# bdaiinstitute/vlfm

Measured on NVIDIA H100. Metric: value-map steps/sec (ITM+cone-fuse), higher is better.
Workload: dtype f16

## Files before the change

### include/vlfm_b200.h

```cpp
#ifndef VLFM_B200_H_
#define VLFM_B200_H_

#include <stddef.h>
#include <stdint.h>

#ifdef __cplusplus
extern "C" {
#endif

#define VLFM_OK 0
#define VLFM_E_INVALID 1
#define VLFM_E_CUDA 2
#define VLFM_E_UNSUPPORTED 3
#define VLFM_E_DRIVER 4

#define VLFM_ST_CAMERA_OFF_GRID 1
#define VLFM_ST_SCATTER_OOB 2
#define VLFM_ST_FRONTIER_OVERFLOW 4

#define VLFM_FUSE_WEIGHTED 0
#define VLFM_FUSE_MAX_CONFIDENCE 1
#define VLFM_FUSE_REPLACE 2
#define VLFM_FUSE_EQUAL 4

// ... 70 lines not shown

int vlfm_preprocess_im2col(const uint8_t* d_img, uint8_t* d_mid, void* d_out, int B, int H, int W, int OH,
                           int OW, int patch, int ldk, const int32_t* d_hbounds, const int32_t* d_hkk,
                           int hksize, const int32_t* d_vbounds, const int32_t* d_vkk, int vksize,
                           const float* h_mean3, const float* h_std3, void* stream);
int vlfm_assemble_tokens(const float* d_patch, const float* d_cls, const float* d_pos, float* d_x, int B,
                         int T, int D, void* stream);
int vlfm_layernorm(const float* d_x, const float* d_gamma, const float* d_beta, void* d_out16, float* d_out32,
                   int rows, int D, int ldx, int ldo16, int ldo32, float eps, void* stream);
int vlfm_attention_f16(const void* d_q, const void* d_k, const void* d_v, void* d_o, int B, int heads, int Nq,
                       int Nk, int hd, int ldq, int ldk, int ldv, int ldo, float scale, void* stream);
#define VLFM_EPI_BIAS_GELU_F16X2 6
#define VLFM_EPI_BIAS_SILU_F16 7
int vlfm_gemm_f16x2(const void* d_A_hi, const void* d_A_lo, const void* d_W_hi, const void* d_W_lo, const float* d_bias, void* d_out,
                    void* d_out_lo, int M, int N, int K, int lda, int ldw, int ldo, int epilogue, void* stream);
int vlfm_gemm_f16x2_resid_ln(const void* d_A_hi, const void* d_A_lo, const void* d_W_hi, const void* d_W_lo, const float* d_bias,
                             float* d_x, int M, int N, int K, int lda, int ldw, int ldx, const float* d_gamma, const float* d_beta,
                             void* d_out_hi, void* d_out_lo, int ld16, float* d_out32, int ld32, float eps, float* d_partials,
                             size_t partial_bytes, void* stream);
int vlfm_layernorm_x2(const float* d_x, const float* d_gamma, const float* d_beta, void* d_out_hi, void* d_out_lo, float* d_out32,
                      int rows, int D, int ldx, int ldo16, int ldo32, float eps, void* stream);
int vlfm_layernorm_reduce_x2(float* d_x, const float* d_partials, int splits, long long split_stride, const float* d_gamma,
                             const float* d_beta, void* d_out_hi, void* d_out_lo, float* d_out32, int rows, int D, int ldx, int ldo16,
                             int ldo32, float eps, void* stream);
int vlfm_split_x2(const float* d_src, void* d_hi, void* d_lo, long long n, void* stream);
int vlfm_attention_f32(const float* d_q, const float* d_k, const float* d_v, void* d_o_hi, void* d_o_lo, int B, int heads, int Nq,
                       int Nk, int hd, int ldq, int ldk, int ldv, int ldo, float scale, void* stream);
int vlfm_itc_head(const float* d_proj, const float* d_text, float* d_out, int B, int Q, int D, void* stream);
int vlfm_itc_head_multi(const float* d_proj, const float* d_text, float* d_out, int B, int P, int Q, int D, int ldo, void* stream);
int vlfm_im2col_f16(const void* d_x16, int ldx, void* d_col16, int B, int H, int W, int C, int k, int stride, int ldk, void* stream);
// ... 137 lines not shown
```

### vlfm_b200/_lib.py

```python
from __future__ import annotations

import ctypes as C
import os

_HERE = os.path.dirname(os.path.abspath(__file__))
LIB_PATH = os.path.join(_HERE, "libvlfm_b200.so")

VLFM_OK = 0
ST_CAMERA_OFF_GRID = 1
ST_SCATTER_OOB = 2
ST_FRONTIER_OVERFLOW = 4
FUSE_WEIGHTED, FUSE_MAX_CONFIDENCE, FUSE_REPLACE, FUSE_EQUAL = 0, 1, 2, 4
EPI_BIAS_F16, EPI_BIAS_GELU_F16, EPI_BIAS_RESID_F32, EPI_BIAS_F32, EPI_BIAS_RELU_F16 = 0, 1, 2, 3, 4
EPI_BIAS_GELU_F16X2 = 6
EPI_BIAS_SILU_F16 = 7
EPI_CLUSTER_SPLIT = 256
DRAW_LINE, DRAW_CIRCLE, DRAW_RECORD_INTS = 0, 1, 8


class ValueParams(C.Structure):
    _fields_ = [
        ("H", C.c_int32), ("W", C.c_int32), ("G", C.c_int32), ("C", C.c_int32), ("R", C.c_int32),
        ("ppm", C.c_int32), ("depth_scale", C.c_float), ("depth_offset", C.c_float),
        ("decision_threshold", C.c_float), ("fusion", C.c_int32), ("rows_per_tile", C.c_int32),
# ... 37 lines not shown
    "vlfm_cast_f32_f16": (C.c_int, [_P, _P, C.c_long, _P]),
    "vlfm_cast_addpos_f16": (C.c_int, [_P, _P, _P, _P, C.c_long, _P]),
    "vlfm_msda_fused": (C.c_int, [_P, _P, C.c_int, C.c_int, _P, C.c_int, _P, C.c_int, C.c_int, C.c_int, C.c_int, C.c_int, C.c_int, _P, _P]),
    "vlfm_holes_workspace_bytes": (C.c_int, [C.c_int, C.c_int, C.POINTER(C.c_size_t)]),
    "vlfm_fill_small_holes": (C.c_int, [_P, C.c_int, C.c_int, C.c_double, _P, _P, _P, _P]),
    "vlfm_gemm_f16": (C.c_int, [_P, _P, _P, _P, C.c_int, C.c_int, C.c_int, C.c_int, C.c_int, C.c_int, C.c_int, _P]),
    "vlfm_gemm_csplit_plan": (C.c_int, [C.c_int, C.c_int, C.c_int, _P, _P, _P]),
    "vlfm_gemm_f16_resid_ln": (C.c_int, [_P, _P, _P, _P] + [C.c_int] * 6 + [_P, _P, _P, C.c_int, _P, C.c_int, C.c_float, _P, C.c_size_t, _P]),
    "vlfm_layernorm_reduce": (C.c_int, [_P, _P, C.c_int, C.c_longlong, _P, _P, _P, _P] + [C.c_int] * 5 + [C.c_float, _P]),
    "vlfm_preprocess_im2col": (C.c_int, [_P, _P, _P] + [C.c_int] * 7 + [_P, _P, C.c_int, _P, _P, C.c_int,
                                         C.POINTER(C.c_float), C.POINTER(C.c_float), _P]),
    "vlfm_assemble_tokens": (C.c_int, [_P, _P, _P, _P, C.c_int, C.c_int, C.c_int, _P]),
    "vlfm_layernorm": (C.c_int, [_P, _P, _P, _P, _P, C.c_int, C.c_int, C.c_int, C.c_int, C.c_int, C.c_float, _P]),
    "vlfm_attention_f16": (C.c_int, [_P, _P, _P, _P] + [C.c_int] * 9 + [C.c_float, _P]),
    "vlfm_gemm_f16x2": (C.c_int, [_P] * 7 + [C.c_int] * 7 + [_P]),
    "vlfm_gemm_f16x2_resid_ln": (C.c_int, [_P] * 6 + [C.c_int] * 6 + [_P, _P, _P, _P, C.c_int, _P, C.c_int, C.c_float, _P, C.c_size_t, _P]),
    "vlfm_layernorm_x2": (C.c_int, [_P] * 6 + [C.c_int] * 5 + [C.c_float, _P]),
    "vlfm_layernorm_reduce_x2": (C.c_int, [_P, _P, C.c_int, C.c_longlong, _P, _P, _P, _P, _P] + [C.c_int] * 5 + [C.c_float, _P]),
    "vlfm_split_x2": (C.c_int, [_P, _P, _P, C.c_longlong, _P]),
    "vlfm_attention_f32": (C.c_int, [_P] * 5 + [C.c_int] * 9 + [C.c_float, _P]),
    "vlfm_swin_patch_im2col": (C.c_int, [_P, _P, C.c_int, C.c_int, C.c_int, C.POINTER(C.c_float), C.POINTER(C.c_float), _P]),
    "vlfm_swin_window_attention": (C.c_int, [_P, _P, _P, _P] + [C.c_int] * 6 + [_P]),
    "vlfm_swin_patch_merge": (C.c_int, [_P, _P, C.c_int, C.c_int, C.c_int, C.c_int, _P]),
    "vlfm_explore_workspace_bytes": (C.c_int, [C.c_int, C.POINTER(C.c_size_t)]),
    "vlfm_explore_update": (C.c_int, [C.c_int, _P, _P, C.c_int, C.c_int, C.c_double, C.c_double, C.c_double, C.c_double, C.c_int, _P, _P, _P, _P, _P]),
    "vlfm_explore_env_record_bytes": (C.c_size_t, []),
    "vlfm_explore_batch_workspace_bytes": (C.c_int, [C.c_int, C.c_int, C.POINTER(C.c_size_t)]),
    "vlfm_explore_update_batch": (C.c_int, [C.c_int, C.c_int, C.POINTER(ExploreEnv), _P, _P, _P, _P, _P, _P, C.c_size_t, _P, C.c_size_t, _P]),
    "vlfm_explore_prepare_batch": (C.c_int, [C.c_int, C.c_int, C.POINTER(ExploreEnv), _P, _P, _P, _P, _P, _P, C.c_size_t, _P, C.c_size_t]),
    "vlfm_explore_launch_batch": (C.c_int, [C.c_int, C.c_int, _P, _P, _P]),
# ... 97 lines not shown
```

### vlfm_b200/csrc/gemm_wgmma.cu

```cuda
#include <cuda.h>
#include <cuda_fp16.h>
#include <math.h>
#include <stdlib.h>

#include "common.cuh"

namespace vlfm {

constexpr int BM = 128;
constexpr int BK = 64;
constexpr int GEMM_THREADS = 384;
constexpr int GEMM_CONSUMERS = 256;

__device__ __forceinline__ void mbar_expect_tx(uint32_t bar, uint32_t bytes) {
  asm volatile("mbarrier.arrive.expect_tx.shared::cta.b64 _, [%0], %1;" ::"r"(bar), "r"(bytes) : "memory");
}
__device__ __forceinline__ void mbar_arrive(uint32_t bar) {
  asm volatile("mbarrier.arrive.shared::cta.b64 _, [%0];" ::"r"(bar) : "memory");
}
__device__ __forceinline__ void tma_load_2d(uint32_t dst, const CUtensorMap* map, int x, int y, uint32_t bar) {
  asm volatile(
      "cp.async.bulk.tensor.2d.shared::cluster.global.mbarrier::complete_tx::bytes [%0], [%1, {%3, %4}], [%2];"
      ::"r"(dst), "l"(map), "r"(bar), "r"(x), "r"(y) : "memory");
}
// ... 51 lines not shown
  }
};
#undef VLFM_D16
#undef VLFM_D4

struct GemmArgs {
  const float* bias;
  void* out;
  int M, N, K, ldo, epi;
  int kb_per_split;
  long long split_stride;
  const __half* a_tail; int lda, tail_rows, tail_row0;
  void* out_lo;
  int a_box_rows;
  SplitK sk;
};
constexpr int GEMM_TAIL_MAX = 2;
static_assert(SK_SLAB_ROWS == BM + GEMM_TAIL_MAX && SK_TILE == BM, "stream-K slab = one 128 x 128 tile + its tail rows");
constexpr int GEMM_TAIL_KMAX = 6144;

__device__ __forceinline__ float gelu_erf(float x) { return 0.5f * x * (1.f + erff(x * 0.70710678118654752f)); }
__device__ __forceinline__ float silu(float x) { return x / (1.f + expf(-x)); }

__device__ __forceinline__ void epilogue_store2(const GemmArgs& g, int row, int n, float v0, float v1, bool pair, bool split) {
  const size_t idx = (size_t)row * g.ldo + n;
  if (g.epi == VLFM_EPI_BIAS_F16 || g.epi == VLFM_EPI_BIAS_GELU_F16 || g.epi == VLFM_EPI_BIAS_RELU_F16 || g.epi == VLFM_EPI_BIAS_GELU_F16X2) {
    if (g.epi == VLFM_EPI_BIAS_GELU_F16 || g.epi == VLFM_EPI_BIAS_GELU_F16X2) { v0 = gelu_erf(v0); v1 = gelu_erf(v1); }
    else if (g.epi == VLFM_EPI_BIAS_RELU_F16) { v0 = fmaxf(v0, 0.f); v1 = fmaxf(v1, 0.f); }
    __half* o = reinterpret_cast<__half*>(g.out) + idx;
    const __half2 h = __floats2half2_rn(v0, v1);
    if (pair) *reinterpret_cast<__half2*>(o) = h; else o[0] = __low2half(h);
    if (g.epi == VLFM_EPI_BIAS_GELU_F16X2) {
      const float2 f = __half22float2(h);
      const __half2 l = __floats2half2_rn((v0 - f.x) * X2_SCALE, (v1 - f.y) * X2_SCALE);
// ... 420 lines not shown
      const int rows = CS_BM + g.tail_rows, r0 = rank * rows / s_cl, r1 = (rank + 1) * rows / s_cl;
      const uint32_t base = smem_u32(part);
      for (int i = et; i < (r1 - r0) * (BN / 2); i += CS_CONSUMERS) {
        const int row = r0 + i / (BN / 2), c = (i % (BN / 2)) * 2, n = n_blk * BN + c;
        if (n >= g.N) continue;
        const uint32_t off = base + (uint32_t)(row * LDP + c) * 4;
        float2 sum = ld_peer_f2(off, 0);
        for (int p = 1; p < s_cl; ++p) { const float2 v = ld_peer_f2(off, p); sum.x += v.x; sum.y += v.y; }
        epilogue_store2(g, row, n, sum.x + sbias[c], sum.y + sbias[c + 1], n + 1 < g.N, false);
      }
    }
    cluster_sync_all();
  }
}

template <int BN, int STAGES>
__global__ void __launch_bounds__(GEMM_THREADS, 1)
gemm_f16x2_wgmma_kernel(const __grid_constant__ CUtensorMap tmA, const __grid_constant__ CUtensorMap tmAl,
                        const __grid_constant__ CUtensorMap tmB, const __grid_constant__ CUtensorMap tmBl, GemmArgs g) {
  constexpr uint32_t A_BYTES = BM * BK * 2, B_BYTES = BN * BK * 2;

  extern __shared__ uint8_t smem_raw[];
  uint8_t* sA = smem_align_1024(smem_raw);
  uint8_t* sAl = sA + STAGES * A_BYTES;
  uint8_t* sB = sAl + STAGES * A_BYTES;
  uint8_t* sBl = sB + STAGES * B_BYTES;
  uint64_t* bars = reinterpret_cast<uint64_t*>(sBl + STAGES * B_BYTES);
  const uint32_t full0 = smem_u32(bars), empty0 = smem_u32(bars + STAGES);
  float* sbias = reinterpret_cast<float*>(bars + 2 * STAGES);

  pdl_trigger();
// ... 35 lines not shown
        tma_load_2d(smem_u32(sA + s * A_BYTES), &tmA, (kb_begin + kb) * BK, m_blk * BM, full0 + 8 * s);
        tma_load_2d(smem_u32(sAl + s * A_BYTES), &tmAl, (kb_begin + kb) * BK, m_blk * BM, full0 + 8 * s);
        tma_load_2d(smem_u32(sB + s * B_BYTES), &tmB, (kb_begin + kb) * BK, n_blk * BN, full0 + 8 * s);
        tma_load_2d(smem_u32(sBl + s * B_BYTES), &tmBl, (kb_begin + kb) * BK, n_blk * BN, full0 + 8 * s);
        if (++s == STAGES) { s = 0; ph ^= 1; }
      }
    }
  } else if (warp >= 4) {
    const int wg = (warp >> 2) - 1, wq = warp & 3;
    const int et = threadIdx.x - (GEMM_THREADS - GEMM_CONSUMERS);
    const int wg_row0 = m_blk * BM + wg * 64;
    const bool active = wg_row0 < g.M;
    if (et < BN) { const int n = n_blk * BN + et; sbias[et] = (g.bias && n < g.N) ? __ldg(g.bias + n) : 0.f; }
    asm volatile("bar.sync 1, 256;" ::: "memory");
    pdl_wait();
    if (!active) {
      int s = 0; uint32_t ph = 0;
      for (int kb = 0; kb < num_k; ++kb) {
        mbar_wait(full0 + 8 * s, ph);
        __syncwarp();
        if (lane == 0) mbar_arrive(empty0 + 8 * s);
        if (++s == STAGES) { s = 0; ph ^= 1; }
      }
      return;
    }
    float acc[BN / 2], corr[BN / 2];
#pragma unroll
    for (int i = 0; i < BN / 2; ++i) { acc[i] = 0.f; corr[i] = 0.f; }
    int s = 0; uint32_t ph = 0;
    for (int kb = 0; kb < num_k; ++kb) {
      mbar_wait(full0 + 8 * s, ph);
      const uint32_t wg_off = (uint32_t)wg * (64 * BK * 2);
      const uint32_t a0 = smem_u32(sA + s * A_BYTES) + wg_off, al0 = smem_u32(sAl + s * A_BYTES) + wg_off;
      const uint32_t b0 = smem_u32(sB + s * B_BYTES), bl0 = smem_u32(sBl + s * B_BYTES);
      wg_fence();
#pragma unroll
      for (int k = 0; k < BK / 16; ++k) {
        const uint64_t da = wgmma_desc_k128(a0 + k * 32), dal = wgmma_desc_k128(al0 + k * 32);
        const uint64_t db = wgmma_desc_k128(b0 + k * 32), dbl = wgmma_desc_k128(bl0 + k * 32);
        const uint32_t first = (kb > 0 || k > 0) ? 1u : 0u;
        Wgmma<BN>::mma(acc, da, db, first);
        Wgmma<BN>::mma(corr, dal, db, first);
        Wgmma<BN>::mma(corr, da, dbl, 1u);
      }
      wg_commit();
      wg_wait<1>();
      if (kb > 0) {
        __syncwarp();
        if (lane == 0) mbar_arrive(empty0 + 8 * (s == 0 ? STAGES - 1 : s - 1));
      }
      if (++s == STAGES) { s = 0; ph ^= 1; }
    }
    wg_wait<0>();
#pragma unroll
    for (int i = 0; i < BN / 2; ++i) acc[i] = fmaf(corr[i], 1.f / X2_SCALE, acc[i]);
    epilogue_frag<BN>(acc, wg_row0 + wq * 16, n_blk, g, split, blockIdx.z == 0, sbias);
  }
}

typedef CUresult (*EncodeTiledFn)(CUtensorMap*, CUtensorMapDataType, cuuint32_t, void*, const cuuint64_t*,
                                  const cuuint64_t*, const cuuint32_t*, const cuuint32_t*, CUtensorMapInterleave,
                                  CUtensorMapSwizzle, CUtensorMapL2promotion, CUtensorMapFloatOOBfill);

static EncodeTiledFn get_encode() {
  static EncodeTiledFn fn = nullptr;
  static bool tried = false;
  if (!tried) {
    tried = true;
    void* p = nullptr;
    cudaDriverEntryPointQueryResult q;
    if (cudaGetDriverEntryPoint("cuTensorMapEncodeTiled", &p, cudaEnableDefault, &q) == cudaSuccess &&
// ... 32 lines not shown
  if (!configured) {
    rc = check_cuda(cudaFuncSetAttribute(gemm_f16_wgmma_kernel<BN, STAGES, SILU>, cudaFuncAttributeMaxDynamicSharedMemorySize, (int)smem), "cudaFuncSetAttribute(gemm)");
    if (rc) return rc;
    configured = true;
  }
  const int num_k = (g.K + BK - 1) / BK;
  dim3 grid((g.N + BN - 1) / BN, g.tail_rows > 0 ? g.M / BM : (g.M + BM - 1) / BM, (num_k + g.kb_per_split - 1) / g.kb_per_split);
  if (g.sk.ctas > 0) grid = dim3(g.sk.ctas);
  rc = check_cuda(launch_pdl(gemm_f16_wgmma_kernel<BN, STAGES, SILU>, grid, dim3(GEMM_THREADS), smem, st, ta, tb, g), "gemm_f16_wgmma_kernel");
  if (rc) return rc;
  count_launch();
  return VLFM_OK;
}


template <int BN, int STAGES>
static int launch_gemm_x2(const CUtensorMap& ta, const CUtensorMap& tal, const void* W, const void* Wl, int ldw, const GemmArgs& g, cudaStream_t st) {
  CUtensorMap tb, tbl;
  int rc = make_map(&tb, W, g.N, g.K, ldw, BN);
  if (!rc) rc = make_map(&tbl, Wl, g.N, g.K, ldw, BN);
  if (rc) return rc;
  constexpr size_t smem = (size_t)STAGES * 2 * (BM * BK * 2 + BN * BK * 2) + 2 * STAGES * 8 + 1024 + BN * 4;
  static_assert(smem <= 227 * 1024, "x2 GEMM stage ring exceeds the 227 KB a block may use");
  static bool configured = false;
  if (!configured) {
    rc = check_cuda(cudaFuncSetAttribute(gemm_f16x2_wgmma_kernel<BN, STAGES>, cudaFuncAttributeMaxDynamicSharedMemorySize, (int)smem), "cudaFuncSetAttribute(gemm x2)");
    if (rc) return rc;
    configured = true;
  }
  const int num_k = (g.K + BK - 1) / BK;
  dim3 grid((g.N + BN - 1) / BN, (g.M + BM - 1) / BM, (num_k + g.kb_per_split - 1) / g.kb_per_split);
  rc = check_cuda(launch_pdl(gemm_f16x2_wgmma_kernel<BN, STAGES>, grid, dim3(GEMM_THREADS), smem, st, ta, tal, tb, tbl, g), "gemm_f16x2_wgmma_kernel");
  if (rc) return rc;
  count_launch();
  return VLFM_OK;
}

template <int BN, int STAGES>
struct Csplit {
  static constexpr size_t smem = (size_t)STAGES * (CS_BM * BK * 2 + BN * BK * 2) + 2 * STAGES * 8 + 1024 + BN * 4 +
                                 (size_t)GEMM_TAIL_MAX * GEMM_TAIL_KMAX * 2;
  static_assert(smem <= 227 * 1024, "cluster-split GEMM stage ring exceeds the 227 KB a block may use");
  static int configure() {
    static int rc = -1;
    if (rc < 0) rc = check_cuda(cudaFuncSetAttribute(gemm_f16_csplit_wgmma_kernel<BN, STAGES>, cudaFuncAttributeMaxDynamicSharedMemorySize, (int)smem),
                                "cudaFuncSetAttribute(gemm csplit)");
    return rc;
// ... 220 lines not shown
                                      int ld16, float* d_out32, int ld32, float eps, float* d_partials, size_t partial_bytes, void* stream) {
  if (!d_A || !d_W || !d_x || !d_gamma || !d_beta || (!d_out16 && !d_out32) || M < 1 || N < 1 || K < 1) {
    set_error("vlfm_gemm_f16_resid_ln: bad argument"); return VLFM_E_INVALID; }
  if ((K & 7) || (lda & 7) || (ldw & 7) || (ldx & 7) || (N & 3) || (ld16 & 3) || (ld32 & 3) || ((uintptr_t)d_A & 15) || ((uintptr_t)d_W & 15) ||
      ((uintptr_t)d_x & 15) || ((uintptr_t)d_partials & 15)) { set_error("vlfm_gemm_f16_resid_ln: alignment (K, strides %% 8; N %% 4; 16-byte pointers)"); return VLFM_E_INVALID; }
  int rc = layernorm_check("vlfm_gemm_f16_resid_ln", d_x, d_gamma, d_beta, d_out16, nullptr, d_out32, N, ldx, ld16, ld32);
  if (rc) return rc;
  GemmArgs g{d_bias, d_x, M, N, K, ldx, VLFM_EPI_BIAS_RESID_F32, (K + BK - 1) / BK, 0, nullptr, 0, 0, 0, nullptr, BM};
  SplitK layout;
  rc = gemm_dispatch(d_A, d_W, M, N, K, lda, ldw, g, stream, d_partials, partial_bytes, &layout, d_partials != nullptr);
  if (rc) return rc;
  if (layout.splits != 1) return layernorm_reduce_impl(d_x, d_partials, layout, d_gamma, d_beta, d_out16, nullptr, d_out32, M, N, ldx, ld16, ld32, eps, stream);
  return vlfm_layernorm(d_x, d_gamma, d_beta, d_out16, d_out32, M, N, ldx, ld16, ld32, eps, stream);
}

static int gemm_x2_dispatch(const void* d_A_hi, const void* d_A_lo, const void* d_W_hi, const void* d_W_lo, int M, int N, int K, int lda, int ldw,
                            GemmArgs g, void* stream, float* d_partials, size_t partial_bytes, int* splits_out) {
  if (splits_out) *splits_out = 1;
  const int rem = M % BM;
  if (M > BM && rem >= 1 && rem <= 32 && (g.epi == VLFM_EPI_BIAS_F32 || g.epi == VLFM_EPI_BIAS_GELU_F16X2)) {
    const int m0 = M - rem;
    GemmArgs g0 = g; g0.M = m0;
    int rc0 = gemm_x2_dispatch(d_A_hi, d_A_lo, d_W_hi, d_W_lo, m0, N, K, lda, ldw, g0, stream, nullptr, 0, nullptr);
    if (rc0) return rc0;
    GemmArgs g1 = g; g1.M = rem;
    const size_t esz = g.epi == VLFM_EPI_BIAS_F32 ? 4 : 2;
    g1.out = (uint8_t*)g.out + (size_t)m0 * g.ldo * esz;
    if (g.out_lo) g1.out_lo = (uint8_t*)g.out_lo + (size_t)m0 * g.ldo * 2;
    return gemm_x2_dispatch((const __half*)d_A_hi + (size_t)m0 * lda, (const __half*)d_A_lo + (size_t)m0 * lda, d_W_hi, d_W_lo, rem, N, K, lda, ldw, g1,
                            stream, nullptr, 0, nullptr);
  }
  CUtensorMap ta, tal;
  g.a_box_rows = M <= 32 ? 32 : (M <= 64 ? 64 : BM);
  int rc = make_map(&ta, d_A_hi, M, K, lda, g.a_box_rows);
  if (!rc) rc = make_map(&tal, d_A_lo, M, K, lda, g.a_box_rows);
  if (rc) return rc;
  const int mt = (M + BM - 1) / BM, num_k = (K + BK - 1) / BK;
  int bn = 32;
  if (mt >= 2 && N >= 4096) bn = 128;
  else if ((long)mt * ((N + 63) / 64) >= 96) bn = 64;
  const int tiles = mt * ((N + bn - 1) / bn);
  int sp = 1;
  if (g.epi == VLFM_EPI_BIAS_RESID_F32 && d_partials) {
    sp = sm_count() / tiles; if (sp > num_k / 3) sp = num_k / 3; if (sp > 8) sp = 8; if (sp < 1) sp = 1;
  }
  g.kb_per_split = (num_k + sp - 1) / sp;
  const int launched = (num_k + g.kb_per_split - 1) / g.kb_per_split;
  if (launched > 1) {
    if ((size_t)launched * (size_t)M * (size_t)N * 4 > partial_bytes) { g.kb_per_split = num_k; }
    else { g.epi = VLFM_EPI_PARTIAL_F32; g.out = d_partials; g.ldo = N; g.split_stride = (long long)M * N; if (splits_out) *splits_out = launched; }
  }
  cudaStream_t st = (cudaStream_t)stream;
  if (bn == 128) return launch_gemm_x2<128, 3>(ta, tal, d_W_hi, d_W_lo, ldw, g, st);
  if (bn == 64) return launch_gemm_x2<64, 4>(ta, tal, d_W_hi, d_W_lo, ldw, g, st);
  return launch_gemm_x2<32, 5>(ta, tal, d_W_hi, d_W_lo, ldw, g, st);
}

static int x2_args_ok(const char* who, const void* a, const void* al, const void* w, const void* wl, const void* out, int M, int N, int K, int lda, int ldw, int ldo) {
  if (!a || !al || !w || !wl || !out || M < 1 || N < 1 || K < 1) { set_error("%s: bad argument", who); return VLFM_E_INVALID; }
  if ((K & 7) || (lda & 7) || (ldw & 7) || (ldo & 7) || ((uintptr_t)a & 15) || ((uintptr_t)al & 15) || ((uintptr_t)w & 15) || ((uintptr_t)wl & 15) || ((uintptr_t)out & 15)) {
    set_error("%s: K, lda, ldw, ldo must be multiples of 8 and pointers 16-byte aligned", who); return VLFM_E_INVALID; }
  return VLFM_OK;
}

extern "C" int vlfm_gemm_f16x2(const void* d_A_hi, const void* d_A_lo, const void* d_W_hi, const void* d_W_lo, const float* d_bias, void* d_out,
                               void* d_out_lo, int M, int N, int K, int lda, int ldw, int ldo, int epilogue, void* stream) {
  int rc = x2_args_ok("vlfm_gemm_f16x2", d_A_hi, d_A_lo, d_W_hi, d_W_lo, d_out, M, N, K, lda, ldw, ldo);
  if (rc) return rc;
  if (epilogue != VLFM_EPI_BIAS_F32 && epilogue != VLFM_EPI_BIAS_RESID_F32 && epilogue != VLFM_EPI_BIAS_GELU_F16X2) {
    set_error("vlfm_gemm_f16x2: epilogue %d unsupported (fp32, fp32 residual, GELU x2)", epilogue); return VLFM_E_INVALID; }
  if (epilogue == VLFM_EPI_BIAS_GELU_F16X2 && (!d_out_lo || ((uintptr_t)d_out_lo & 15))) { set_error("vlfm_gemm_f16x2: d_out_lo missing / unaligned"); return VLFM_E_INVALID; }
  GemmArgs g{d_bias, d_out, M, N, K, ldo, epilogue, (K + BK - 1) / BK, 0, nullptr, 0, 0, 0, d_out_lo, BM};
  return gemm_x2_dispatch(d_A_hi, d_A_lo, d_W_hi, d_W_lo, M, N, K, lda, ldw, g, stream, nullptr, 0, nullptr);
}

extern "C" int vlfm_layernorm_x2(const float* d_x, const float* d_gamma, const float* d_beta, void* d_out_hi, void* d_out_lo, float* d_out32,
                                 int rows, int D, int ldx, int ldo16, int ldo32, float eps, void* stream);
extern "C" int vlfm_layernorm_reduce_x2(float* d_x, const float* d_partials, int splits, long long split_stride, const float* d_gamma,
                                        const float* d_beta, void* d_out_hi, void* d_out_lo, float* d_out32, int rows, int D, int ldx, int ldo16,
                                        int ldo32, float eps, void* stream);

extern "C" int vlfm_gemm_f16x2_resid_ln(const void* d_A_hi, const void* d_A_lo, const void* d_W_hi, const void* d_W_lo, const float* d_bias,
                                        float* d_x, int M, int N, int K, int lda, int ldw, int ldx, const float* d_gamma, const float* d_beta,
                                        void* d_out_hi, void* d_out_lo, int ld16, float* d_out32, int ld32, float eps, float* d_partials,
                                        size_t partial_bytes, void* stream) {
  int rc = x2_args_ok("vlfm_gemm_f16x2_resid_ln", d_A_hi, d_A_lo, d_W_hi, d_W_lo, d_x, M, N, K, lda, ldw, ldx);
  if (rc) return rc;
  if (!d_gamma || !d_beta || !d_out_hi || !d_out_lo || (N & 3) || (ld16 & 3) || (ld32 & 3) || ((uintptr_t)d_partials & 15)) {
// ... 11 lines not shown
```

### vlfm_b200/vlm/blip2_engine.py

```python
from __future__ import annotations

import ctypes
import math
from typing import Dict, List, Sequence, Tuple

import numpy as np
import torch

from .. import _lib
from ..utils.cuda_graph import GraphCache, default_use_graph
from . import dense
from .blip2_config import Blip2Dims
from .preprocess import CLIP_MEAN, CLIP_STD, bicubic_tables

F16, F32 = torch.float16, torch.float32


def partials_floats(dims: Blip2Dims, max_batch: int) -> int:
    rows = max_batch * dims.tokens
    return max(8 * min(rows, 1024), 3 * rows) * max(dims.v_hidden, dims.q_hidden)


class Blip2ITCEngine:
    def __init__(self, dims: Blip2Dims, state_dict: Dict[str, torch.Tensor], device="cuda", max_batch: int = 1) -> None:
        if not torch.cuda.is_available():
            raise _lib.VlfmError("vlfm_b200 needs a CUDA device (no CPU fallback)")
        self.lib = _lib.load()
        self.d = dims
        self.dev = torch.device(device)
        self.max_batch = max_batch
        self.use_graph = default_use_graph()
        self.graphs = GraphCache()
        self._tables: Dict[Tuple[int, int], Tuple[torch.Tensor, ...]] = {}
        self._mean = (ctypes.c_float * 3)(*CLIP_MEAN)
        self._std = (ctypes.c_float * 3)(*CLIP_STD)
        self._load(state_dict)
        self._alloc(max_batch)
        self.text_feat = torch.zeros(dims.proj, dtype=F32, device=self.dev)
        self.fuse_ln = True
        self._partials = torch.empty(partials_floats(dims, max_batch), dtype=F32, device=self.dev)
        self._fold_layer0()
        self._many_out: Dict[int, torch.Tensor] = {}
        self.generation = 0

    def _load(self, sd: Dict[str, torch.Tensor]) -> None:
        d, dev = self.d, self.dev

        def h(t):
            return t.to(dev, F16).contiguous()

        def f(t):
            return t.to(dev, F32).contiguous()

        def lo(t):
            t = t.to(dev, F32)
# ... 81 lines not shown
        self.q_h16 = e(B * Q, H)
        self.q_h_lo = e(B * Q, H)
        self.q_qkv32 = e(B * Q, 3 * H, dt=F32)
        self.q_q32 = e(B * Q, H, dt=F32)
        self.q_ao = e(B * Q, H)
        self.q_ao_lo = e(B * Q, H)
        self.q_f = e(B * Q, I)
        self.q_f_lo = e(B * Q, I)
        self.q_proj = e(B * Q, d.proj, dt=F32)
        self.out = torch.zeros(B, dtype=F32, device=dev)

    def _gemm(self, a, w, bias, epi, out):
        dense.gemm_f16(a, w, bias, epi | _lib.EPI_CLUSTER_SPLIT, out)

    def _gemm_x2(self, a, al, w, wl, bias, epi, out, out_lo=None):
        dense.gemm_f16x2(a, al, w, wl, bias, epi, out, out_lo)

    def _gemm_resid_ln(self, a, w, bias, x, g, b, out16, out32, eps):
        if not self.fuse_ln:
            self._gemm(a, w, bias, _lib.EPI_BIAS_RESID_F32, x)
            dense.layernorm(x, g, b, eps, out16, out32)
            return
        dense.gemm_f16_resid_ln(a, w, bias, x, g, b, eps, out16, out32, partials=self._partials)

    def _gemm_x2_resid_ln(self, a, al, w, wl, bias, x, g, b, out_hi, out_lo, out32, eps):
        if not self.fuse_ln:
            self._gemm_x2(a, al, w, wl, bias, _lib.EPI_BIAS_RESID_F32, x)
            dense.layernorm_x2(x, g, b, eps, out_hi, out_lo, out32)
            return
        dense.gemm_f16x2_resid_ln(a, al, w, wl, bias, x, g, b, eps, out_hi, out_lo, out32, partials=self._partials)

# ... 146 lines not shown
```

### vlfm_b200/vlm/dense.py

```python
from __future__ import annotations

from typing import Optional

import torch

from .. import _lib

F16, F32 = torch.float16, torch.float32
Tensor = torch.Tensor


def gemm_f16(a: Tensor, w: Tensor, bias: Optional[Tensor], epilogue: int, out: Optional[Tensor] = None,
             rows: Optional[int] = None) -> Tensor:
    M, K = a.shape
    if rows is not None:
        M = rows
    if out is None:
        epi = epilogue & ~_lib.EPI_CLUSTER_SPLIT
        assert epi != _lib.EPI_BIAS_RESID_F32, "the residual epilogue updates a caller-given stream"
        out = torch.empty((M, w.shape[0]), dtype=F32 if epi == _lib.EPI_BIAS_F32 else F16, device=a.device)
    rc = _lib.load().vlfm_gemm_f16(a.data_ptr(), w.data_ptr(), _lib.ptr(bias), out.data_ptr(), M, w.shape[0], K, a.stride(0),
                                   w.stride(0), out.stride(0), epilogue, _lib.stream_ptr())
    _lib.check(rc, "vlfm_gemm_f16")
    return out
# ... 2 lines not shown
def gemm_f16_resid_ln(a: Tensor, w: Tensor, bias: Optional[Tensor], x: Tensor, gamma: Tensor, beta: Tensor, eps: float,
                      out16: Optional[Tensor] = None, out32: Optional[Tensor] = None, partials: Optional[Tensor] = None,
                      rows: Optional[int] = None) -> None:
    M, K = a.shape
    if rows is not None:
        M = rows
    ws, ws_bytes = (None, 0) if partials is None else (partials.data_ptr(), partials.numel() * 4)
    rc = _lib.load().vlfm_gemm_f16_resid_ln(a.data_ptr(), w.data_ptr(), _lib.ptr(bias), x.data_ptr(), M, w.shape[0], K, a.stride(0),
                                            w.stride(0), x.stride(0), gamma.data_ptr(), beta.data_ptr(),
                                            _lib.ptr(out16), 0 if out16 is None else out16.stride(0),
                                            _lib.ptr(out32), 0 if out32 is None else out32.stride(0), eps, ws, ws_bytes, _lib.stream_ptr())
    _lib.check(rc, "vlfm_gemm_f16_resid_ln")


def gemm_f16x2(a: Tensor, a_lo: Tensor, w: Tensor, w_lo: Tensor, bias: Optional[Tensor], epilogue: int, out: Tensor,
               out_lo: Optional[Tensor] = None) -> None:
    M, K = a.shape
    rc = _lib.load().vlfm_gemm_f16x2(a.data_ptr(), a_lo.data_ptr(), w.data_ptr(), w_lo.data_ptr(), _lib.ptr(bias), out.data_ptr(),
                                     _lib.ptr(out_lo), M, w.shape[0], K, a.stride(0), w.stride(0), out.stride(0), epilogue,
                                     _lib.stream_ptr())
    _lib.check(rc, "vlfm_gemm_f16x2")


def gemm_f16x2_resid_ln(a: Tensor, a_lo: Tensor, w: Tensor, w_lo: Tensor, bias: Optional[Tensor], x: Tensor, gamma: Tensor,
                        beta: Tensor, eps: float, out_hi: Tensor, out_lo: Tensor, out32: Optional[Tensor] = None,
                        partials: Optional[Tensor] = None) -> None:
    M, K = a.shape
    ws, ws_bytes = (None, 0) if partials is None else (partials.data_ptr(), partials.numel() * 4)
    rc = _lib.load().vlfm_gemm_f16x2_resid_ln(a.data_ptr(), a_lo.data_ptr(), w.data_ptr(), w_lo.data_ptr(), _lib.ptr(bias), x.data_ptr(),
                                              M, w.shape[0], K, a.stride(0), w.stride(0), x.stride(0), gamma.data_ptr(), beta.data_ptr(),
                                              out_hi.data_ptr(), out_lo.data_ptr(), out_hi.stride(0),
                                              _lib.ptr(out32), 0 if out32 is None else out32.stride(0), eps, ws, ws_bytes, _lib.stream_ptr())
    _lib.check(rc, "vlfm_gemm_f16x2_resid_ln")


def layernorm(x: Tensor, gamma: Tensor, beta: Tensor, eps: float, out16=None, out32=None):
# ... 78 lines not shown
```

Measured before the change: 233.9.

## Add split-K ticket reduction and fused tail rows to x2 GEMM

Adds a split-K variant of the hi/lo f16x2 WGMMA GEMM for small-M (<=32) problems. It uses a bytes-based planner to choose tile width and split count, and the last-arriving CTA reduces per-split fp32 slabs through an atomic ticket counter. It also folds 1-2 leftover rows beyond a multiple of 128 into the last M tile, where they are computed with scalar FMAs from shared-memory weights, so no separate tail launch is needed. This cuts launch count and raises SM occupancy for skinny GEMMs, at the cost of workspace traffic, extra shared memory and more complex synchronization.

```diff
diff --git a/include/vlfm_b200.h b/include/vlfm_b200.h
--- a/include/vlfm_b200.h
+++ b/include/vlfm_b200.h
@@ -108,6 +108,9 @@
 #define VLFM_EPI_BIAS_SILU_F16 7
 int vlfm_gemm_f16x2(const void* d_A_hi, const void* d_A_lo, const void* d_W_hi, const void* d_W_lo, const float* d_bias, void* d_out,
                     void* d_out_lo, int M, int N, int K, int lda, int ldw, int ldo, int epilogue, void* stream);
+int vlfm_gemm_f16x2_split(const void* d_A_hi, const void* d_A_lo, const void* d_W_hi, const void* d_W_lo, const float* d_bias, void* d_out,
+                          void* d_out_lo, int M, int N, int K, int lda, int ldw, int ldo, int epilogue, float* d_partials,
+                          size_t partial_bytes, unsigned int* d_tickets, int n_tickets, void* stream);
 int vlfm_gemm_f16x2_resid_ln(const void* d_A_hi, const void* d_A_lo, const void* d_W_hi, const void* d_W_lo, const float* d_bias,
                              float* d_x, int M, int N, int K, int lda, int ldw, int ldx, const float* d_gamma, const float* d_beta,
                              void* d_out_hi, void* d_out_lo, int ld16, float* d_out32, int ld32, float eps, float* d_partials,
diff --git a/vlfm_b200/_lib.py b/vlfm_b200/_lib.py
--- a/vlfm_b200/_lib.py
+++ b/vlfm_b200/_lib.py
@@ -75,6 +75,7 @@
     "vlfm_layernorm": (C.c_int, [_P, _P, _P, _P, _P, C.c_int, C.c_int, C.c_int, C.c_int, C.c_int, C.c_float, _P]),
     "vlfm_attention_f16": (C.c_int, [_P, _P, _P, _P] + [C.c_int] * 9 + [C.c_float, _P]),
     "vlfm_gemm_f16x2": (C.c_int, [_P] * 7 + [C.c_int] * 7 + [_P]),
+    "vlfm_gemm_f16x2_split": (C.c_int, [_P] * 7 + [C.c_int] * 7 + [_P, C.c_size_t, _P, C.c_int, _P]),
     "vlfm_gemm_f16x2_resid_ln": (C.c_int, [_P] * 6 + [C.c_int] * 6 + [_P, _P, _P, _P, C.c_int, _P, C.c_int, C.c_float, _P, C.c_size_t, _P]),
     "vlfm_layernorm_x2": (C.c_int, [_P] * 6 + [C.c_int] * 5 + [C.c_float, _P]),
     "vlfm_layernorm_reduce_x2": (C.c_int, [_P, _P, C.c_int, C.c_longlong, _P, _P, _P, _P, _P] + [C.c_int] * 5 + [C.c_float, _P]),
diff --git a/vlfm_b200/csrc/gemm_wgmma.cu b/vlfm_b200/csrc/gemm_wgmma.cu
--- a/vlfm_b200/csrc/gemm_wgmma.cu
+++ b/vlfm_b200/csrc/gemm_wgmma.cu
@@ -2,6 +2,7 @@
 #include <cuda_fp16.h>
 #include <math.h>
 #include <stdlib.h>
+#include <string.h>
 
 #include "common.cuh"
 
@@ -89,10 +90,15 @@
   void* out_lo;
   int a_box_rows;
   SplitK sk;
+  float* ws;
+  unsigned int* tickets;
+  const __half* a_tail_lo;
 };
 constexpr int GEMM_TAIL_MAX = 2;
 static_assert(SK_SLAB_ROWS == BM + GEMM_TAIL_MAX && SK_TILE == BM, "stream-K slab = one 128 x 128 tile + its tail rows");
 constexpr int GEMM_TAIL_KMAX = 6144;
+constexpr int X2_RED_ROWS = 32;
+constexpr int X2_TAIL_KMAX = 2048;
 
 __device__ __forceinline__ float gelu_erf(float x) { return 0.5f * x * (1.f + erff(x * 0.70710678118654752f)); }
 __device__ __forceinline__ float silu(float x) { return x / (1.f + expf(-x)); }
@@ -543,7 +549,7 @@
   }
 }
 
-template <int BN, int STAGES>
+template <int BN, int STAGES, bool REDUCE = false, bool TAIL = false>
 __global__ void __launch_bounds__(GEMM_THREADS, 1)
 gemm_f16x2_wgmma_kernel(const __grid_constant__ CUtensorMap tmA, const __grid_constant__ CUtensorMap tmAl,
                         const __grid_constant__ CUtensorMap tmB, const __grid_constant__ CUtensorMap tmBl, GemmArgs g) {
@@ -609,6 +615,26 @@
     if (et < BN) { const int n = n_blk * BN + et; sbias[et] = (g.bias && n < g.N) ? __ldg(g.bias + n) : 0.f; }
     asm volatile("bar.sync 1, 256;" ::: "memory");
     pdl_wait();
+    const bool tail_cta = TAIL && m_blk == (int)gridDim.y - 1;
+    const int f = et >> 1, hk = et & 1;
+    float thh[GEMM_TAIL_MAX], tcr[GEMM_TAIL_MAX];
+    __half* sx = reinterpret_cast<__half*>(sbias + BN);
+    const int kslice = num_k * BK;
+    if constexpr (TAIL) {
+#pragma unroll
+      for (int r = 0; r < GEMM_TAIL_MAX; ++r) { thh[r] = 0.f; tcr[r] = 0.f; }
+      if (tail_cta) {
+        for (int i = et; i < 2 * g.tail_rows * (kslice >> 3); i += GEMM_CONSUMERS) {
+          const int hr = i / (kslice >> 3), c8 = (i - hr * (kslice >> 3)) << 3;
+          const int half = hr / g.tail_rows, r = hr - half * g.tail_rows;
+          const __half* src = half ? g.a_tail_lo : g.a_tail;
+          uint4 xv = make_uint4(0u, 0u, 0u, 0u);
+          if (kb_begin * BK + c8 < g.K) xv = __ldg(reinterpret_cast<const uint4*>(src + (size_t)r * g.lda + kb_begin * BK + c8));
+          *reinterpret_cast<uint4*>(sx + ((size_t)half * GEMM_TAIL_MAX + r) * kslice + c8) = xv;
+        }
+        asm volatile("bar.sync 1, 256;" ::: "memory");
+      }
+    }
     if (!active) {
       int s = 0; uint32_t ph = 0;
       for (int kb = 0; kb < num_k; ++kb) {
@@ -639,6 +665,36 @@
         Wgmma<BN>::mma(corr, da, dbl, 1u);
       }
       wg_commit();
+      if constexpr (TAIL) {
+        if (tail_cta && f < BN) {
+          const uint8_t* wrow = sB + (size_t)s * B_BYTES + (size_t)f * 128;
+          const uint8_t* wlrow = sBl + (size_t)s * B_BYTES + (size_t)f * 128;
+          const int k0 = kb * BK + hk * 32;
+#pragma unroll
+          for (int c = 0; c < 4; ++c) {
+            const int sw = ((hk * 4 + c) ^ (f & 7)) << 4;
+            const uint4 wv = *reinterpret_cast<const uint4*>(wrow + sw), wlv = *reinterpret_cast<const uint4*>(wlrow + sw);
+            const __half2* wh = reinterpret_cast<const __half2*>(&wv);
+            const __half2* wl = reinterpret_cast<const __half2*>(&wlv);
+#pragma unroll
+            for (int r = 0; r < GEMM_TAIL_MAX; ++r) {
+              if (r < g.tail_rows) {
+                const uint4 xv = *reinterpret_cast<const uint4*>(sx + (size_t)r * kslice + k0 + c * 8);
+                const uint4 xlv = *reinterpret_cast<const uint4*>(sx + ((size_t)GEMM_TAIL_MAX + r) * kslice + k0 + c * 8);
+                const __half2* xh = reinterpret_cast<const __half2*>(&xv);
+                const __half2* xl = reinterpret_cast<const __half2*>(&xlv);
+#pragma unroll
+                for (int e = 0; e < 4; ++e) {
+                  const float2 a = __half22float2(xh[e]), al = __half22float2(xl[e]), w = __half22float2(wh[e]), wlo = __half22float2(wl[e]);
+                  thh[r] = fmaf(a.x, w.x, thh[r]); thh[r] = fmaf(a.y, w.y, thh[r]);
+                  tcr[r] = fmaf(al.x, w.x, tcr[r]); tcr[r] = fmaf(al.y, w.y, tcr[r]);
+                  tcr[r] = fmaf(a.x, wlo.x, tcr[r]); tcr[r] = fmaf(a.y, wlo.y, tcr[r]);
+                }
+              }
+            }
+          }
+        }
+      }
       wg_wait<1>();
       if (kb > 0) {
         __syncwarp();
@@ -649,7 +705,54 @@
     wg_wait<0>();
 #pragma unroll
     for (int i = 0; i < BN / 2; ++i) acc[i] = fmaf(corr[i], 1.f / X2_SCALE, acc[i]);
-    epilogue_frag<BN>(acc, wg_row0 + wq * 16, n_blk, g, split, blockIdx.z == 0, sbias);
+    if constexpr (TAIL) {
+      if (tail_cta) {
+#pragma unroll
+        for (int r = 0; r < GEMM_TAIL_MAX; ++r) { thh[r] += __shfl_xor_sync(0xffffffffu, thh[r], 1); tcr[r] += __shfl_xor_sync(0xffffffffu, tcr[r], 1); }
+        const int n = n_blk * BN + f;
+        if (hk == 0 && f < BN && n < g.N) {
+#pragma unroll
+          for (int r = 0; r < GEMM_TAIL_MAX; ++r)
+            if (r < g.tail_rows) epilogue_store2(g, g.tail_row0 + r, n, fmaf(tcr[r], 1.f / X2_SCALE, thh[r]) + sbias[f], 0.f, false, false);
+        }
+      }
+    }
+    if constexpr (!REDUCE) {
+      epilogue_frag<BN>(acc, wg_row0 + wq * 16, n_blk, g, split, blockIdx.z == 0, sbias);
+    } else {
+      __shared__ unsigned int s_ticket;
+      const int tile = n_blk, r_up = wq * 16 + (lane >> 2), cq = (lane & 3) * 2;
+      const size_t tile_off = ((size_t)tile * X2_RED_ROWS + r_up) * BN + cq, split_floats = (size_t)gridDim.x * X2_RED_ROWS * BN;
+      if (wq < 2) {
+        float* slab = g.ws + (size_t)blockIdx.z * split_floats + tile_off;
+#pragma unroll
+        for (int j = 0; j < BN / 8; ++j) {
+          *reinterpret_cast<float2*>(slab + j * 8) = make_float2(acc[4 * j], acc[4 * j + 1]);
+          *reinterpret_cast<float2*>(slab + 8 * BN + j * 8) = make_float2(acc[4 * j + 2], acc[4 * j + 3]);
+        }
+      }
+      __threadfence();
+      asm volatile("bar.sync 2, 128;" ::: "memory");
+      if (et == 0) s_ticket = atomicAdd(g.tickets + tile, 1u);
+      asm volatile("bar.sync 2, 128;" ::: "memory");
+      if (s_ticket != gridDim.z - 1) return;
+      if (et == 0) g.tickets[tile] = 0u;
+      __threadfence();
+      if (wq < 2) {
+#pragma unroll
+        for (int i = 0; i < BN / 2; ++i) acc[i] = 0.f;
+        for (int z = 0; z < (int)gridDim.z; ++z) {
+          const float* slab = g.ws + (size_t)z * split_floats + tile_off;
+#pragma unroll
+          for (int j = 0; j < BN / 8; ++j) {
+            const float2 u = __ldcg(reinterpret_cast<const float2*>(slab + j * 8));
+            const float2 v = __ldcg(reinterpret_cast<const float2*>(slab + 8 * BN + j * 8));
+            acc[4 * j] += u.x; acc[4 * j + 1] += u.y; acc[4 * j + 2] += v.x; acc[4 * j + 3] += v.y;
+          }
+        }
+        epilogue_frag<BN>(acc, wq * 16, n_blk, g, false, true, sbias);
+      }
+    }
   }
 }
 
@@ -712,23 +815,24 @@
 }
 
 
-template <int BN, int STAGES>
+template <int BN, int STAGES, bool REDUCE = false, bool TAIL = false>
 static int launch_gemm_x2(const CUtensorMap& ta, const CUtensorMap& tal, const void* W, const void* Wl, int ldw, const GemmArgs& g, cudaStream_t st) {
   CUtensorMap tb, tbl;
   int rc = make_map(&tb, W, g.N, g.K, ldw, BN);
   if (!rc) rc = make_map(&tbl, Wl, g.N, g.K, ldw, BN);
   if (rc) return rc;
-  constexpr size_t smem = (size_t)STAGES * 2 * (BM * BK * 2 + BN * BK * 2) + 2 * STAGES * 8 + 1024 + BN * 4;
+  constexpr size_t smem = (size_t)STAGES * 2 * (BM * BK * 2 + BN * BK * 2) + 2 * STAGES * 8 + 1024 + BN * 4 +
+                          (TAIL ? (size_t)2 * GEMM_TAIL_MAX * X2_TAIL_KMAX * 2 : 0);
   static_assert(smem <= 227 * 1024, "x2 GEMM stage ring exceeds the 227 KB a block may use");
   static bool configured = false;
   if (!configured) {
-    rc = check_cuda(cudaFuncSetAttribute(gemm_f16x2_wgmma_kernel<BN, STAGES>, cudaFuncAttributeMaxDynamicSharedMemorySize, (int)smem), "cudaFuncSetAttribute(gemm x2)");
+    rc = check_cuda(cudaFuncSetAttribute(gemm_f16x2_wgmma_kernel<BN, STAGES, REDUCE, TAIL>, cudaFuncAttributeMaxDynamicSharedMemorySize, (int)smem), "cudaFuncSetAttribute(gemm x2)");
     if (rc) return rc;
     configured = true;
   }
   const int num_k = (g.K + BK - 1) / BK;
-  dim3 grid((g.N + BN - 1) / BN, (g.M + BM - 1) / BM, (num_k + g.kb_per_split - 1) / g.kb_per_split);
-  rc = check_cuda(launch_pdl(gemm_f16x2_wgmma_kernel<BN, STAGES>, grid, dim3(GEMM_THREADS), smem, st, ta, tal, tb, tbl, g), "gemm_f16x2_wgmma_kernel");
+  dim3 grid((g.N + BN - 1) / BN, TAIL ? g.M / BM : (g.M + BM - 1) / BM, (num_k + g.kb_per_split - 1) / g.kb_per_split);
+  rc = check_cuda(launch_pdl(gemm_f16x2_wgmma_kernel<BN, STAGES, REDUCE, TAIL>, grid, dim3(GEMM_THREADS), smem, st, ta, tal, tb, tbl, g), "gemm_f16x2_wgmma_kernel");
   if (rc) return rc;
   count_launch();
   return VLFM_OK;
@@ -979,10 +1083,31 @@
   return vlfm_layernorm(d_x, d_gamma, d_beta, d_out16, d_out32, M, N, ldx, ld16, ld32, eps, stream);
 }
 
+constexpr int X2_RED_BN = 32;
+constexpr int X2_RED_MIN_KB = 3;
+constexpr double X2_RED_FIXED_BYTES = 16384;
+static bool x2_legacy_plan() {
+  const char* e = getenv("VLFM_X2_PLAN");
+  return e && !strcmp(e, "legacy");
+}
+
 static int gemm_x2_dispatch(const void* d_A_hi, const void* d_A_lo, const void* d_W_hi, const void* d_W_lo, int M, int N, int K, int lda, int ldw,
-                            GemmArgs g, void* stream, float* d_partials, size_t partial_bytes, int* splits_out) {
+                            GemmArgs g, void* stream, float* d_partials, size_t partial_bytes, int* splits_out,
+                            unsigned int* d_tickets = nullptr, int n_tickets = 0) {
   if (splits_out) *splits_out = 1;
   const int rem = M % BM;
+  if (M > BM && rem <= GEMM_TAIL_MAX && rem >= 1 && N >= 4096 && K <= X2_TAIL_KMAX && d_tickets && !x2_legacy_plan() &&
+      (g.epi == VLFM_EPI_BIAS_F32 || g.epi == VLFM_EPI_BIAS_GELU_F16X2)) {
+    CUtensorMap ta, tal;
+    g.a_box_rows = BM;
+    int rc = make_map(&ta, d_A_hi, M - rem, K, lda, BM);
+    if (!rc) rc = make_map(&tal, d_A_lo, M - rem, K, lda, BM);
+    if (rc) return rc;
+    g.a_tail = (const __half*)d_A_hi + (size_t)(M - rem) * lda; g.a_tail_lo = (const __half*)d_A_lo + (size_t)(M - rem) * lda;
+    g.lda = lda; g.tail_rows = rem; g.tail_row0 = M - rem;
+    g.kb_per_split = (K + BK - 1) / BK;
+    return launch_gemm_x2<128, 3, false, true>(ta, tal, d_W_hi, d_W_lo, ldw, g, (cudaStream_t)stream);
+  }
   if (M > BM && rem >= 1 && rem <= 32 && (g.epi == VLFM_EPI_BIAS_F32 || g.epi == VLFM_EPI_BIAS_GELU_F16X2)) {
     const int m0 = M - rem;
     GemmArgs g0 = g; g0.M = m0;
@@ -993,7 +1118,7 @@
     g1.out = (uint8_t*)g.out + (size_t)m0 * g.ldo * esz;
     if (g.out_lo) g1.out_lo = (uint8_t*)g.out_lo + (size_t)m0 * g.ldo * 2;
     return gemm_x2_dispatch((const __half*)d_A_hi + (size_t)m0 * lda, (const __half*)d_A_lo + (size_t)m0 * lda, d_W_hi, d_W_lo, rem, N, K, lda, ldw, g1,
-                            stream, nullptr, 0, nullptr);
+                            stream, d_partials, partial_bytes, nullptr, d_tickets, n_tickets);
   }
   CUtensorMap ta, tal;
   g.a_box_rows = M <= 32 ? 32 : (M <= 64 ? 64 : BM);
@@ -1001,6 +1126,33 @@
   if (!rc) rc = make_map(&tal, d_A_lo, M, K, lda, g.a_box_rows);
   if (rc) return rc;
   const int mt = (M + BM - 1) / BM, num_k = (K + BK - 1) / BK;
+  cudaStream_t st = (cudaStream_t)stream;
+  if (M <= 32 && (g.epi == VLFM_EPI_BIAS_F32 || g.epi == VLFM_EPI_BIAS_GELU_F16X2) && d_partials && d_tickets && !x2_legacy_plan()) {
+    const int sms = sm_count();
+    int best_bn = 0, best_kb = 0;
+    double best = 0.0;
+    const int bns[3] = {128, 64, 32};
+    for (int bn : bns) {
+      const int nt = (N + bn - 1) / bn;
+      for (int s = 1; s <= 8 && s <= num_k; ++s) {
+        const int kb = (num_k + s - 1) / s, launched = (num_k + kb - 1) / kb;
+        if (launched != s) continue;
+        if (s > 1 && (bn != X2_RED_BN || kb < X2_RED_MIN_KB || nt * s > sms || nt > n_tickets ||
+                      (size_t)s * nt * X2_RED_ROWS * bn * 4 > partial_bytes)) continue;
+        double bytes = (double)((nt + sms - 1) / sms) * kb * 2 * (32 + bn) * BK * 2;
+        if (s > 1) bytes += (double)s * 32 * bn * 4 + X2_RED_FIXED_BYTES;
+        if (!best_bn || bytes < best) { best = bytes; best_bn = bn; best_kb = kb; }
+      }
+    }
+    g.kb_per_split = best_kb;
+    if (best_kb < num_k) {
+      g.ws = d_partials; g.tickets = d_tickets;
+      return launch_gemm_x2<X2_RED_BN, 5, true>(ta, tal, d_W_hi, d_W_lo, ldw, g, st);
+    }
+    if (best_bn == 128) return launch_gemm_x2<128, 3>(ta, tal, d_W_hi, d_W_lo, ldw, g, st);
+    if (best_bn == 64) return launch_gemm_x2<64, 4>(ta, tal, d_W_hi, d_W_lo, ldw, g, st);
+    return launch_gemm_x2<32, 5>(ta, tal, d_W_hi, d_W_lo, ldw, g, st);
+  }
   int bn = 32;
   if (mt >= 2 && N >= 4096) bn = 128;
   else if ((long)mt * ((N + 63) / 64) >= 96) bn = 64;
@@ -1015,7 +1167,6 @@
     if ((size_t)launched * (size_t)M * (size_t)N * 4 > partial_bytes) { g.kb_per_split = num_k; }
     else { g.epi = VLFM_EPI_PARTIAL_F32; g.out = d_partials; g.ldo = N; g.split_stride = (long long)M * N; if (splits_out) *splits_out = launched; }
   }
-  cudaStream_t st = (cudaStream_t)stream;
   if (bn == 128) return launch_gemm_x2<128, 3>(ta, tal, d_W_hi, d_W_lo, ldw, g, st);
   if (bn == 64) return launch_gemm_x2<64, 4>(ta, tal, d_W_hi, d_W_lo, ldw, g, st);
   return launch_gemm_x2<32, 5>(ta, tal, d_W_hi, d_W_lo, ldw, g, st);
@@ -1037,6 +1188,20 @@
   if (epilogue == VLFM_EPI_BIAS_GELU_F16X2 && (!d_out_lo || ((uintptr_t)d_out_lo & 15))) { set_error("vlfm_gemm_f16x2: d_out_lo missing / unaligned"); return VLFM_E_INVALID; }
   GemmArgs g{d_bias, d_out, M, N, K, ldo, epilogue, (K + BK - 1) / BK, 0, nullptr, 0, 0, 0, d_out_lo, BM};
   return gemm_x2_dispatch(d_A_hi, d_A_lo, d_W_hi, d_W_lo, M, N, K, lda, ldw, g, stream, nullptr, 0, nullptr);
+}
+
+extern "C" int vlfm_gemm_f16x2_split(const void* d_A_hi, const void* d_A_lo, const void* d_W_hi, const void* d_W_lo, const float* d_bias, void* d_out,
+                                     void* d_out_lo, int M, int N, int K, int lda, int ldw, int ldo, int epilogue, float* d_partials,
+                                     size_t partial_bytes, unsigned int* d_tickets, int n_tickets, void* stream) {
+  int rc = x2_args_ok("vlfm_gemm_f16x2_split", d_A_hi, d_A_lo, d_W_hi, d_W_lo, d_out, M, N, K, lda, ldw, ldo);
+  if (rc) return rc;
+  if (epilogue != VLFM_EPI_BIAS_F32 && epilogue != VLFM_EPI_BIAS_RESID_F32 && epilogue != VLFM_EPI_BIAS_GELU_F16X2) {
+    set_error("vlfm_gemm_f16x2_split: epilogue %d unsupported (fp32, fp32 residual, GELU x2)", epilogue); return VLFM_E_INVALID; }
+  if (epilogue == VLFM_EPI_BIAS_GELU_F16X2 && (!d_out_lo || ((uintptr_t)d_out_lo & 15))) { set_error("vlfm_gemm_f16x2_split: d_out_lo missing / unaligned"); return VLFM_E_INVALID; }
+  if (n_tickets < 0 || ((uintptr_t)d_partials & 15) || ((uintptr_t)d_tickets & 3)) { set_error("vlfm_gemm_f16x2_split: bad workspace / tickets"); return VLFM_E_INVALID; }
+  GemmArgs g{d_bias, d_out, M, N, K, ldo, epilogue, (K + BK - 1) / BK, 0, nullptr, 0, 0, 0, d_out_lo, BM};
+  if (epilogue == VLFM_EPI_BIAS_RESID_F32) return gemm_x2_dispatch(d_A_hi, d_A_lo, d_W_hi, d_W_lo, M, N, K, lda, ldw, g, stream, nullptr, 0, nullptr);
+  return gemm_x2_dispatch(d_A_hi, d_A_lo, d_W_hi, d_W_lo, M, N, K, lda, ldw, g, stream, d_partials, partial_bytes, nullptr, d_tickets, n_tickets);
 }
 
 extern "C" int vlfm_layernorm_x2(const float* d_x, const float* d_gamma, const float* d_beta, void* d_out_hi, void* d_out_lo, float* d_out32,
diff --git a/vlfm_b200/vlm/blip2_engine.py b/vlfm_b200/vlm/blip2_engine.py
--- a/vlfm_b200/vlm/blip2_engine.py
+++ b/vlfm_b200/vlm/blip2_engine.py
@@ -19,6 +19,9 @@
 def partials_floats(dims: Blip2Dims, max_batch: int) -> int:
     rows = max_batch * dims.tokens
     return max(8 * min(rows, 1024), 3 * rows) * max(dims.v_hidden, dims.q_hidden)
+
+
+X2_TICKETS = 1024
 
 
 class Blip2ITCEngine:
@@ -39,6 +42,7 @@
         self.text_feat = torch.zeros(dims.proj, dtype=F32, device=self.dev)
         self.fuse_ln = True
         self._partials = torch.empty(partials_floats(dims, max_batch), dtype=F32, device=self.dev)
+        self._tickets = torch.zeros(X2_TICKETS, dtype=torch.int32, device=self.dev)
         self._fold_layer0()
         self._many_out: Dict[int, torch.Tensor] = {}
         self.generation = 0
@@ -150,7 +154,7 @@
         dense.gemm_f16(a, w, bias, epi | _lib.EPI_CLUSTER_SPLIT, out)
 
     def _gemm_x2(self, a, al, w, wl, bias, epi, out, out_lo=None):
-        dense.gemm_f16x2(a, al, w, wl, bias, epi, out, out_lo)
+        dense.gemm_f16x2(a, al, w, wl, bias, epi, out, out_lo, partials=self._partials, tickets=self._tickets)
 
     def _gemm_resid_ln(self, a, w, bias, x, g, b, out16, out32, eps):
         if not self.fuse_ln:
diff --git a/vlfm_b200/vlm/dense.py b/vlfm_b200/vlm/dense.py
--- a/vlfm_b200/vlm/dense.py
+++ b/vlfm_b200/vlm/dense.py
@@ -40,12 +40,19 @@
 
 
 def gemm_f16x2(a: Tensor, a_lo: Tensor, w: Tensor, w_lo: Tensor, bias: Optional[Tensor], epilogue: int, out: Tensor,
-               out_lo: Optional[Tensor] = None) -> None:
+               out_lo: Optional[Tensor] = None, partials: Optional[Tensor] = None, tickets: Optional[Tensor] = None) -> None:
     M, K = a.shape
-    rc = _lib.load().vlfm_gemm_f16x2(a.data_ptr(), a_lo.data_ptr(), w.data_ptr(), w_lo.data_ptr(), _lib.ptr(bias), out.data_ptr(),
-                                     _lib.ptr(out_lo), M, w.shape[0], K, a.stride(0), w.stride(0), out.stride(0), epilogue,
-                                     _lib.stream_ptr())
-    _lib.check(rc, "vlfm_gemm_f16x2")
+    if partials is None or tickets is None:
+        rc = _lib.load().vlfm_gemm_f16x2(a.data_ptr(), a_lo.data_ptr(), w.data_ptr(), w_lo.data_ptr(), _lib.ptr(bias), out.data_ptr(),
+                                         _lib.ptr(out_lo), M, w.shape[0], K, a.stride(0), w.stride(0), out.stride(0), epilogue,
+                                         _lib.stream_ptr())
+        _lib.check(rc, "vlfm_gemm_f16x2")
+        return
+    rc = _lib.load().vlfm_gemm_f16x2_split(a.data_ptr(), a_lo.data_ptr(), w.data_ptr(), w_lo.data_ptr(), _lib.ptr(bias), out.data_ptr(),
+                                           _lib.ptr(out_lo), M, w.shape[0], K, a.stride(0), w.stride(0), out.stride(0), epilogue,
+                                           partials.data_ptr(), partials.numel() * 4, tickets.data_ptr(), tickets.numel(),
+                                           _lib.stream_ptr())
+    _lib.check(rc, "vlfm_gemm_f16x2_split")
 
 
 def gemm_f16x2_resid_ln(a: Tensor, a_lo: Tensor, w: Tensor, w_lo: Tensor, bias: Optional[Tensor], x: Tensor, gamma: Tensor,
```

Result: no change. 233.2, median of 6 (-0.3%).
